# luo-yining/CFDBench

Hardware: NVIDIA H100
Metric: fno_rollout_steps_per_sec (higher is better)
Workload: dtype bf16

## Files before the change

cfdbench_b200/csrc/fno_block_fused.cu:

```cuda
#include "fno_common.cuh"
#include "tc_common.cuh"
#include "tc_tma.cuh"
#include <math.h>
#include <string.h>

namespace fno {

constexpr int kFzRows = 16;
constexpr int kFzChunks = kH / kFzRows;
constexpr int kFzWgRows = kFzRows / 2;
constexpr int kFzThreads = 9 * 32;
constexpr int kFzProdWarp = 8;
constexpr int kZK = 2 * kM2;
constexpr int kImgK = 2 * kKX;
constexpr size_t kYmImgBytes = 147456;
constexpr uint32_t kFzStage = 4 * 6144;
constexpr int kFzFFloats = 2 * (2 * kFzRows) * kImgK;
constexpr int kFzEFloats = 2 * kW * kZK;
constexpr uint32_t kFzZtFloats = kC * kZK;
constexpr uint32_t kLboF = (2 * kFzRows / 8) * 128;
constexpr uint32_t kLboE = (kW / 8) * 128;
constexpr uint32_t kLboO = (kC / 8) * 128;
constexpr uint32_t kFzBoxW = kW, kFzBoxH = 1, kFzBoxC = kC;
constexpr uint32_t kFzRowBytes = kFzBoxW * kFzBoxH * kFzBoxC * 2;
constexpr int kFzXSlots = 4;
constexpr uint32_t kFzW0Bytes = kC * kC * 2;

__host__ __device__ constexpr int fz_x_slot(int n) { return n % kFzXSlots; }
__host__ __device__ constexpr uint32_t fz_x_parity(int n) { return static_cast<uint32_t>(n / kFzXSlots) & 1u; }

struct FzSmem {
  alignas(1024) unsigned char x[2][kFzXSlots][kFzRowBytes];
  alignas(1024) unsigned char st[2][2][kFzRowBytes];
  alignas(128) unsigned char y[2][kFzStage];
  alignas(128) float zt[kFzRows][2][kFzZtFloats];
  alignas(128) float f_hi[kFzFFloats / 2];
  alignas(128) float f_lo[kFzFFloats / 2];
  alignas(128) float e_hi[kFzEFloats / 2];
  alignas(128) float e_lo[kFzEFloats / 2];
  alignas(128) unsigned char w0[3][kFzW0Bytes];
  alignas(16) float bias[kC];
  alignas(8) uint64_t y_full[2], y_free[2];
  alignas(8) uint64_t x_full[2][kFzXSlots];
};
static_assert(sizeof(FzSmem) <= 232448, "block_fused_kernel: shared memory over the per-block opt-in limit");

__device__ __forceinline__ uint32_t sw128_bf16_offset(int line, int e) {
  return static_cast<uint32_t>(line * 128 + ((((e >> 3) ^ line) & 7) << 4) + (e & 7) * 2);
}

__global__ void __launch_bounds__(kFzThreads, 1)
    block_fused_kernel(const __grid_constant__ CUtensorMap x_map, const __grid_constant__ CUtensorMap out_map,
                       const unsigned char* __restrict__ img, const float* __restrict__ w0t,
                       const float* __restrict__ bias, const float* __restrict__ etab, const float* __restrict__ ftab,
                       int batch) {
  extern __shared__ __align__(1024) unsigned char smem_raw[];
  FzSmem& sm = *reinterpret_cast<FzSmem*>(smem_raw);
  if ((smem_u32(smem_raw) & 1023u) != 0) __trap();
  const int tid = threadIdx.x, lane = tid & 31, warp = tc::warp_index_uniform();
  const int chunk = blockIdx.x % kFzChunks, b0 = blockIdx.x / kFzChunks, bstride = gridDim.x / kFzChunks;
  const int n_units = b0 < batch ? (batch - b0 + bstride - 1) / bstride : 0;

  if (tid == 0) {
    for (int i = 0; i < 2; ++i) {
      mbar_init(&sm.y_full[i], 1);
      mbar_init(&sm.y_free[i], 4);
      for (int s = 0; s < kFzXSlots; ++s) mbar_init(&sm.x_full[i][s], 1);
    }
    fence_mbar_init();
  }
  for (int e = tid; e < kFzFFloats / 2; e += kFzThreads) {
    sm.f_hi[e] = __ldg(ftab + chunk * kFzFFloats + e);
    sm.f_lo[e] = __ldg(ftab + chunk * kFzFFloats + kFzFFloats / 2 + e);
  }
  for (int e = tid; e < kFzEFloats / 2; e += kFzThreads) {
    sm.e_hi[e] = __ldg(etab + e);
    sm.e_lo[e] = __ldg(etab + kFzEFloats / 2 + e);
  }
  for (int e = tid; e < kC * kC; e += kFzThreads) {
    const int i = e / kC, o = e % kC;
    const float w = w0t[e];
    const __nv_bfloat16 t1 = __float2bfloat16_rn(w);
    const float r1 = w - __bfloat162float(t1);
    const __nv_bfloat16 t2 = __float2bfloat16_rn(r1);
    const __nv_bfloat16 t3 = __float2bfloat16_rn(r1 - __bfloat162float(t2));
    const uint32_t off = static_cast<uint32_t>(((i >> 3) * (kC / 8) + (o >> 3)) * 128 + (o & 7) * 16 + (i & 7) * 2);
    *reinterpret_cast<__nv_bfloat16*>(sm.w0[0] + off) = t1;
    *reinterpret_cast<__nv_bfloat16*>(sm.w0[1] + off) = t2;
    *reinterpret_cast<__nv_bfloat16*>(sm.w0[2] + off) = t3;
  }
  if (tid < kC) sm.bias[tid] = bias != nullptr ? bias[tid] : 0.f;
  tc::fence_proxy_async_smem();
  __syncthreads();
  pdl_wait();
  pdl_launch_dependents();

  if (warp == kFzProdWarp) {
    if (lane < 2) {
      const int s = lane;
      for (int u = 0; u < n_units; ++u) {
        const unsigned char* src = img + static_cast<size_t>(b0 + u * bstride) * kYmImgBytes;
        for (int pi = 0; pi < 3; ++pi) {
          const int p = s + 2 * pi, f = 3 * u + pi;
          if (f >= 1) mbar_wait(&sm.y_free[s], (f - 1) & 1);
          mbar_expect_tx(&sm.y_full[s], kFzStage);
          bulk_g2s(sm.y[s], src + p * (kFzStage / 2), kFzStage / 2, &sm.y_full[s]);
          bulk_g2s(sm.y[s] + kFzStage / 2, src + kYmImgBytes / 2 + p * (kFzStage / 2), kFzStage / 2, &sm.y_full[s]);
        }
      }
    }
    return;
  }

  const int g = warp >> 2, wq = warp & 3, q = lane & 3, t = tid & 127;
  const int m0 = 16 * wq + (lane >> 2);
  const int n_fills = kFzWgRows * n_units;
  auto x_fill = [&](int n) {
    const int u = n / kFzWgRows, r = n % kFzWgRows, s = fz_x_slot(n);
    mbar_expect_tx(&sm.x_full[g][s], kFzRowBytes);
    tma_load_3d(sm.x[g][s], &x_map, 0, kFzRows * chunk + g + 2 * r, (b0 + u * bstride) * kC, &sm.x_full[g][s]);
  };
  if (t == 0)
    for (int n = 0; n < kFzXSlots && n < n_fills; ++n) x_fill(n);
  const uint32_t w0_s = tc::smem_addr(sm.w0[0]);

  for (int u = 0; u < n_units; ++u) {
    const int b = b0 + u * bstride;
    for (int pi = 0; pi < 3; ++pi) {
      const int p = g + 2 * pi, f = 3 * u + pi;
      mbar_wait(&sm.y_full[g], f & 1);
      uint32_t a_hi[6][4], a_lo[6][4];
#pragma unroll
      for (int ks = 0; ks < kImgK / 8; ++ks)
#pragma unroll
        for (int r = 0; r < 4; ++r) {
          const int m = m0 + 8 * (r & 1), kk = 8 * ks + q + 4 * (r >> 1), o = m & 31;
          const uint32_t off = (m >> 5) * 6144 + kk * 128 + (((o >> 3) ^ (kk & 3)) << 5) + (o & 7) * 4;
          a_hi[ks][r] = *reinterpret_cast<const uint32_t*>(sm.y[g] + off);
          a_lo[ks][r] = *reinterpret_cast<const uint32_t*>(sm.y[g] + kFzStage / 2 + off);
        }
      float acc[16];
      tc::wg_fence();
#pragma unroll
      for (int pass = 0; pass < 3; ++pass) {
        const uint32_t fb = tc::smem_addr(pass == 2 ? sm.f_lo : sm.f_hi);
#pragma unroll
        for (int ks = 0; ks < kImgK / 8; ++ks)
          tc::wg_tf32_rs_n32(acc, pass == 1 ? a_lo[ks] : a_hi[ks], tc::make_smem_desc(fb + ks * 2 * kLboF, kLboF, 128),
                             (pass | ks) ? 1u : 0u);
      }
      tc::wg_commit();
      __syncwarp();
      if (lane == 0) mbar_arrive(&sm.y_free[g]);
      tc::wg_wait<0>();
      tc::wg_fence_acc(acc);
      if (pi == 0) tc::named_barrier(1, 256);
#pragma unroll
      for (int hh = 0; hh < 2; ++hh) {
        const int m = m0 + 8 * hh, ky = 2 * p + (m >> 5), o = m & 31;
#pragma unroll
        for (int i = 0; i < 4; ++i)
#pragma unroll
          for (int e = 0; e < 2; ++e) {
            float v = acc[4 * i + 2 * hh + e];
            if (ky == 0 && e == 1) v = sm.bias[o];
            float hi, lo;
            tc::split_tf32(v, hi, lo);
            const uint32_t off = tc::kmajor_offset(o, 2 * ky + e, kC) / 4;
            sm.zt[4 * i + q][0][off] = hi;
            sm.zt[4 * i + q][1][off] = lo;
          }
      }
    }
    tc::fence_proxy_async_smem();
    tc::named_barrier(1, 256);

    float acc[2][16];
#pragma unroll
    for (int r = 0; r <= kFzWgRows; ++r) {
      if (r < kFzWgRows) {
        const int n = kFzWgRows * u + r, hl = g + 2 * r;
        mbar_wait(&sm.x_full[g][fz_x_slot(n)], fz_x_parity(n));
        tc::wg_fence();
        const uint32_t a_e[3] = {tc::smem_addr(sm.e_hi), tc::smem_addr(sm.e_lo), tc::smem_addr(sm.e_hi)};
        const uint32_t b_z[3] = {tc::smem_addr(sm.zt[hl][0]), tc::smem_addr(sm.zt[hl][0]), tc::smem_addr(sm.zt[hl][1])};
#pragma unroll
        for (int pass = 0; pass < 3; ++pass)
#pragma unroll
          for (int ks = 0; ks < kZK / 8; ++ks)
            tc::wg_tf32_ss_n32(acc[r & 1], tc::make_smem_desc(a_e[pass] + ks * 2 * kLboE, kLboE, 128),
                               tc::make_smem_desc(b_z[pass] + ks * 2 * kLboO, kLboO, 128), (pass | ks) ? 1u : 0u);
        tc::wg_fence();
        const uint32_t a_x = tc::smem_addr(sm.x[g][fz_x_slot(n)]);
#pragma unroll
        for (int term = 0; term < 3; ++term)
#pragma unroll
          for (int ks = 0; ks < kC / 16; ++ks)
            tc::wg_bf16_ss_n32_mn_a(acc[r & 1], tc::make_smem_desc_sw128_mn(a_x + ks * 2048),
                                    tc::make_smem_desc(w0_s + term * kFzW0Bytes + ks * 2 * kLboO, kLboO, 128), 1u);
        tc::wg_commit();
      }
      if (r == 0) continue;
      const int rr = r - 1, h = kFzRows * chunk + g + 2 * rr;
      float* d = acc[rr & 1];
      if (r < kFzWgRows) {
        tc::wg_wait<1>();
      } else {
        tc::wg_wait<0>();
      }
      tc::wg_fence_acc(acc[rr & 1]);
      unsigned char* stile = sm.st[g][rr & 1];
#pragma unroll
      for (int i = 0; i < 4; ++i)
#pragma unroll
        for (int hh = 0; hh < 2; ++hh) {
          const float2 v = gelu_erf2(make_float2(d[4 * i + 2 * hh], d[4 * i + 2 * hh + 1]));
          const int w = m0 + 8 * hh, o = 8 * i + 2 * q;
          *reinterpret_cast<__nv_bfloat16*>(stile + sw128_bf16_offset(o, w)) = __float2bfloat16_rn(v.x);
          *reinterpret_cast<__nv_bfloat16*>(stile + sw128_bf16_offset(o + 1, w)) = __float2bfloat16_rn(v.y);
        }
      tc::fence_proxy_async_smem();
      if (t == 0) bulk_wait_group_read<0>();
      tc::named_barrier(2 + g, 128);
      if (t == 0) {
        tma_store_3d(&out_map, stile, 0, h, b * kC);
        bulk_commit_group();
        const int nf = kFzWgRows * u + rr + kFzXSlots;
        if (nf < n_fills) x_fill(nf);
      }
    }
  }
  if (t == 0) bulk_wait_group<0>();
}

void c2r_operand_table(float* host, double s0, double s1);

static float fz_round_tf32_host(double v) {
  float f = static_cast<float>(v);
  uint32_t u;
  memcpy(&u, &f, 4);
  u = (u + 0x1000u) & 0xffffe000u;
  memcpy(&f, &u, 4);
  return f;
}

struct FzTables {
  float* etab = nullptr;
  float* ftab = nullptr;
  int n_sm = 0;
  bool configured = false;
};
static FzTables g_fz[64];

static cudaError_t fz_ensure(int dev, cudaStream_t stream) {
  FzTables& t = g_fz[dev];
  if (t.configured) return cudaSuccess;
  const double two_pi = 6.283185307179586476925286766559;
  static float h_e[kFzEFloats];
  static float h_f[kFzChunks * kFzFFloats];
  c2r_operand_table(h_e, 1.0 / kHW, 2.0 / kHW);
  for (int c = 0; c < kFzChunks; ++c)
    for (int n = 0; n < 2 * kFzRows; ++n) {
      const int h = kFzRows * c + (n >> 1), ri = n & 1;
      for (int k = 0; k < kImgK; ++k) {
        const int rip = k & 1, kxi = 2 * ((k % 24) >> 1) + k / 24, kx = kxi < kM1 ? kxi : kxi + (kH - kKX);
        const double ang = two_pi * ((kx * h) % 64) / 64.0;
        const double val = (ri == rip) ? cos(ang) : (ri == 0 ? -sin(ang) : sin(ang));
        const float hi = fz_round_tf32_host(val);
        const uint32_t off = tc::kmajor_offset(n, k, 2 * kFzRows) / 4;
        h_f[c * kFzFFloats + off] = hi;
        h_f[c * kFzFFloats + kFzFFloats / 2 + off] = fz_round_tf32_host(val - static_cast<double>(hi));
      }
    }
  cudaError_t e = cudaMalloc(&t.etab, sizeof(h_e));
  if (e != cudaSuccess) return e;
  e = cudaMalloc(&t.ftab, sizeof(h_f));
  if (e != cudaSuccess) return e;
  e = cudaMemcpyAsync(t.etab, h_e, sizeof(h_e), cudaMemcpyHostToDevice, stream);
  if (e != cudaSuccess) return e;
  e = cudaMemcpyAsync(t.ftab, h_f, sizeof(h_f), cudaMemcpyHostToDevice, stream);
  if (e != cudaSuccess) return e;
  e = cudaStreamSynchronize(stream);
  if (e != cudaSuccess) return e;
  e = cudaFuncSetAttribute(block_fused_kernel, cudaFuncAttributeMaxDynamicSharedMemorySize, (int)sizeof(FzSmem));
  if (e != cudaSuccess) return e;
  e = cudaDeviceGetAttribute(&t.n_sm, cudaDevAttrMultiProcessorCount, dev);
  if (e != cudaSuccess) return e;
  t.configured = true;
  return cudaSuccess;
}

void block_fused_release(int dev) {
  if (dev < 0 || dev >= 64) return;
  FzTables& t = g_fz[dev];
  if (t.etab) cudaFree(t.etab);
  if (t.ftab) cudaFree(t.ftab);
  t = FzTables();
}

cudaError_t launch_block_fused(const void* ym_img, const void* x, const float* w0t, const float* bias, void* out, int batch,
                               cudaStream_t stream) {
  int dev = 0;
  cudaError_t e = cudaGetDevice(&dev);
  if (e != cudaSuccess) return e;
  if (dev < 0 || dev >= 64) return cudaErrorInvalidDevice;
  e = fz_ensure(dev, stream);
  if (e != cudaSuccess) return e;
  if ((reinterpret_cast<uintptr_t>(x) & 15) || (reinterpret_cast<uintptr_t>(ym_img) & 15) ||
      (reinterpret_cast<uintptr_t>(out) & 15))
    return cudaErrorMisalignedAddress;
  CUtensorMap x_map, out_map;
  const uint64_t planes = static_cast<uint64_t>(batch) * kC;
  e = make_tma_map_3d(&x_map, CU_TENSOR_MAP_DATA_TYPE_BFLOAT16, 2, x, kW, kH, planes, kFzBoxW, kFzBoxH, kFzBoxC);
  if (e != cudaSuccess) return e;
  e = make_tma_map_3d(&out_map, CU_TENSOR_MAP_DATA_TYPE_BFLOAT16, 2, out, kW, kH, planes, kFzBoxW, kFzBoxH, kFzBoxC);
  if (e != cudaSuccess) return e;
  const int slots_max = g_fz[dev].n_sm / kFzChunks;
  const int slots = batch < slots_max ? batch : slots_max;
  return launch_chained(block_fused_kernel, dim3(kFzChunks * slots), dim3(kFzThreads), sizeof(FzSmem), stream, x_map,
                        out_map, static_cast<const unsigned char*>(ym_img), w0t, bias,
                        static_cast<const float*>(g_fz[dev].etab), static_cast<const float*>(g_fz[dev].ftab), batch);
}

}
```

cfdbench_b200/csrc/tc_common.cuh:

```cuda
#pragma once
#include <cuda_runtime.h>
#include <stdint.h>

namespace fno {
namespace tc {

__device__ __forceinline__ uint32_t smem_addr(const void* p) {
  return static_cast<uint32_t>(__cvta_generic_to_shared(p));
}

__device__ __forceinline__ int warp_index_uniform() {
  return __shfl_sync(0xffffffffu, static_cast<int>(threadIdx.x >> 5), 0);
}

__device__ __forceinline__ void named_barrier(int id, int count) {
  asm volatile("bar.sync %0, %1;" ::"r"(id), "r"(count) : "memory");
}

__device__ __forceinline__ void fence_proxy_async_smem() {
  asm volatile("fence.proxy.async.shared::cta;" ::: "memory");
}

__device__ __forceinline__ uint64_t make_smem_desc(uint32_t saddr, uint32_t lbo_bytes, uint32_t sbo_bytes) {
  uint64_t d = 0;
  d |= static_cast<uint64_t>((saddr & 0x3FFFFu) >> 4);
  d |= static_cast<uint64_t>((lbo_bytes >> 4) & 0x3FFFu) << 16;
  d |= static_cast<uint64_t>((sbo_bytes >> 4) & 0x3FFFu) << 32;
  return d;
}
__device__ __forceinline__ uint64_t make_smem_desc_sw128(uint32_t saddr) {
  return make_smem_desc(saddr, 16, 1024) | (static_cast<uint64_t>(1) << 62);
}
__device__ __forceinline__ uint64_t make_smem_desc_sw128_mn(uint32_t saddr) {
  return make_smem_desc(saddr, 16, 1024) | (static_cast<uint64_t>(1) << 62);
}

__device__ __forceinline__ void wg_fence() { asm volatile("wgmma.fence.sync.aligned;" ::: "memory"); }
__device__ __forceinline__ void wg_commit() { asm volatile("wgmma.commit_group.sync.aligned;" ::: "memory"); }
template <int kPending>
__device__ __forceinline__ void wg_wait() { asm volatile("wgmma.wait_group.sync.aligned %0;" ::"n"(kPending) : "memory"); }
template <int N>
__device__ __forceinline__ void wg_fence_acc(float (&d)[N]) {
#pragma unroll
  for (int i = 0; i < N; ++i) asm volatile("" : "+f"(d[i])::"memory");
}

__device__ __forceinline__ void wg_tf32_ss_n32(float* d, uint64_t a, uint64_t b, uint32_t acc) {
  asm volatile(
      "{\n.reg .pred p;\nsetp.ne.b32 p, %18, 0;\n"
      "wgmma.mma_async.sync.aligned.m64n32k8.f32.tf32.tf32 {%0, %1, %2, %3, %4, %5, %6, %7, %8, %9, %10, %11, %12, %13, %14, %15}, %16, %17, p, 1, 1;\n}\n"
      : "+f"(d[0]), "+f"(d[1]), "+f"(d[2]), "+f"(d[3]), "+f"(d[4]), "+f"(d[5]), "+f"(d[6]), "+f"(d[7]), "+f"(d[8]), "+f"(d[9]), "+f"(d[10]), "+f"(d[11]), "+f"(d[12]), "+f"(d[13]), "+f"(d[14]), "+f"(d[15])
      : "l"(a), "l"(b), "r"(acc)
      : "memory");
}
__device__ __forceinline__ void wg_tf32_ss_n128(float* d, uint64_t a, uint64_t b, uint32_t acc) {
  asm volatile(
      "{\n.reg .pred p;\nsetp.ne.b32 p, %66, 0;\n"
      "wgmma.mma_async.sync.aligned.m64n128k8.f32.tf32.tf32 {%0, %1, %2, %3, %4, %5, %6, %7, %8, %9, %10, %11, %12, %13, %14, %15, %16, %17, %18, %19, %20, %21, %22, %23, %24, %25, %26, %27, %28, %29, %30, %31, %32, %33, %34, %35, %36, %37, %38, %39, %40, %41, %42, %43, %44, %45, %46, %47, %48, %49, %50, %51, %52, %53, %54, %55, %56, %57, %58, %59, %60, %61, %62, %63}, %64, %65, p, 1, 1;\n}\n"
      : "+f"(d[0]), "+f"(d[1]), "+f"(d[2]), "+f"(d[3]), "+f"(d[4]), "+f"(d[5]), "+f"(d[6]), "+f"(d[7]), "+f"(d[8]), "+f"(d[9]), "+f"(d[10]), "+f"(d[11]), "+f"(d[12]), "+f"(d[13]), "+f"(d[14]), "+f"(d[15]), "+f"(d[16]), "+f"(d[17]), "+f"(d[18]), "+f"(d[19]), "+f"(d[20]), "+f"(d[21]), "+f"(d[22]), "+f"(d[23]), "+f"(d[24]), "+f"(d[25]), "+f"(d[26]), "+f"(d[27]), "+f"(d[28]), "+f"(d[29]), "+f"(d[30]), "+f"(d[31]), "+f"(d[32]), "+f"(d[33]), "+f"(d[34]), "+f"(d[35]), "+f"(d[36]), "+f"(d[37]), "+f"(d[38]), "+f"(d[39]), "+f"(d[40]), "+f"(d[41]), "+f"(d[42]), "+f"(d[43]), "+f"(d[44]), "+f"(d[45]), "+f"(d[46]), "+f"(d[47]), "+f"(d[48]), "+f"(d[49]), "+f"(d[50]), "+f"(d[51]), "+f"(d[52]), "+f"(d[53]), "+f"(d[54]), "+f"(d[55]), "+f"(d[56]), "+f"(d[57]), "+f"(d[58]), "+f"(d[59]), "+f"(d[60]), "+f"(d[61]), "+f"(d[62]), "+f"(d[63])
      : "l"(a), "l"(b), "r"(acc)
      : "memory");
}
__device__ __forceinline__ void wg_bf16_ss_n72(float* d, uint64_t a, uint64_t b, uint32_t acc) {
  asm volatile(
      "{\n.reg .pred p;\nsetp.ne.b32 p, %38, 0;\n"
      "wgmma.mma_async.sync.aligned.m64n72k16.f32.bf16.bf16 {%0, %1, %2, %3, %4, %5, %6, %7, %8, %9, %10, %11, %12, %13, %14, %15, %16, %17, %18, %19, %20, %21, %22, %23, %24, %25, %26, %27, %28, %29, %30, %31, %32, %33, %34, %35}, %36, %37, p, 1, 1, 0, 0;\n}\n"
      : "+f"(d[0]), "+f"(d[1]), "+f"(d[2]), "+f"(d[3]), "+f"(d[4]), "+f"(d[5]), "+f"(d[6]), "+f"(d[7]), "+f"(d[8]), "+f"(d[9]), "+f"(d[10]), "+f"(d[11]), "+f"(d[12]), "+f"(d[13]), "+f"(d[14]), "+f"(d[15]), "+f"(d[16]), "+f"(d[17]), "+f"(d[18]), "+f"(d[19]), "+f"(d[20]), "+f"(d[21]), "+f"(d[22]), "+f"(d[23]), "+f"(d[24]), "+f"(d[25]), "+f"(d[26]), "+f"(d[27]), "+f"(d[28]), "+f"(d[29]), "+f"(d[30]), "+f"(d[31]), "+f"(d[32]), "+f"(d[33]), "+f"(d[34]), "+f"(d[35])
      : "l"(a), "l"(b), "r"(acc)
      : "memory");
}
__device__ __forceinline__ void wg_bf16_ss_n32_mn_a(float* d, uint64_t a, uint64_t b, uint32_t acc) {
  asm volatile(
      "{\n.reg .pred p;\nsetp.ne.b32 p, %18, 0;\n"
      "wgmma.mma_async.sync.aligned.m64n32k16.f32.bf16.bf16 {%0, %1, %2, %3, %4, %5, %6, %7, %8, %9, %10, %11, %12, %13, %14, %15}, %16, %17, p, 1, 1, 1, 0;\n}\n"
      : "+f"(d[0]), "+f"(d[1]), "+f"(d[2]), "+f"(d[3]), "+f"(d[4]), "+f"(d[5]), "+f"(d[6]), "+f"(d[7]), "+f"(d[8]), "+f"(d[9]), "+f"(d[10]), "+f"(d[11]), "+f"(d[12]), "+f"(d[13]), "+f"(d[14]), "+f"(d[15])
      : "l"(a), "l"(b), "r"(acc)
      : "memory");
}
__device__ __forceinline__ void wg_tf32_rs_n32(float* d, const uint32_t* a, uint64_t b, uint32_t acc) {
  asm volatile(
      "{\n.reg .pred p;\nsetp.ne.b32 p, %21, 0;\n"
      "wgmma.mma_async.sync.aligned.m64n32k8.f32.tf32.tf32 {%0, %1, %2, %3, %4, %5, %6, %7, %8, %9, %10, %11, %12, %13, %14, %15}, {%16, %17, %18, %19}, %20, p, 1, 1;\n}\n"
      : "+f"(d[0]), "+f"(d[1]), "+f"(d[2]), "+f"(d[3]), "+f"(d[4]), "+f"(d[5]), "+f"(d[6]), "+f"(d[7]), "+f"(d[8]), "+f"(d[9]), "+f"(d[10]), "+f"(d[11]), "+f"(d[12]), "+f"(d[13]), "+f"(d[14]), "+f"(d[15])
      : "r"(a[0]), "r"(a[1]), "r"(a[2]), "r"(a[3]), "l"(b), "r"(acc)
      : "memory");
}
__device__ __forceinline__ void wg_tf32_rs_n48(float* d, const uint32_t* a, uint64_t b, uint32_t acc) {
  asm volatile(
      "{\n.reg .pred p;\nsetp.ne.b32 p, %29, 0;\n"
      "wgmma.mma_async.sync.aligned.m64n48k8.f32.tf32.tf32 {%0, %1, %2, %3, %4, %5, %6, %7, %8, %9, %10, %11, %12, %13, %14, %15, %16, %17, %18, %19, %20, %21, %22, %23}, {%24, %25, %26, %27}, %28, p, 1, 1;\n}\n"
      : "+f"(d[0]), "+f"(d[1]), "+f"(d[2]), "+f"(d[3]), "+f"(d[4]), "+f"(d[5]), "+f"(d[6]), "+f"(d[7]), "+f"(d[8]), "+f"(d[9]), "+f"(d[10]), "+f"(d[11]), "+f"(d[12]), "+f"(d[13]), "+f"(d[14]), "+f"(d[15]), "+f"(d[16]), "+f"(d[17]), "+f"(d[18]), "+f"(d[19]), "+f"(d[20]), "+f"(d[21]), "+f"(d[22]), "+f"(d[23])
      : "r"(a[0]), "r"(a[1]), "r"(a[2]), "r"(a[3]), "l"(b), "r"(acc)
      : "memory");
}
__device__ __forceinline__ void wg_tf32_rs_n64(float* d, const uint32_t* a, uint64_t b, uint32_t acc) {
  asm volatile(
      "{\n.reg .pred p;\nsetp.ne.b32 p, %37, 0;\n"
      "wgmma.mma_async.sync.aligned.m64n64k8.f32.tf32.tf32 {%0, %1, %2, %3, %4, %5, %6, %7, %8, %9, %10, %11, %12, %13, %14, %15, %16, %17, %18, %19, %20, %21, %22, %23, %24, %25, %26, %27, %28, %29, %30, %31}, {%32, %33, %34, %35}, %36, p, 1, 1;\n}\n"
      : "+f"(d[0]), "+f"(d[1]), "+f"(d[2]), "+f"(d[3]), "+f"(d[4]), "+f"(d[5]), "+f"(d[6]), "+f"(d[7]), "+f"(d[8]), "+f"(d[9]), "+f"(d[10]), "+f"(d[11]), "+f"(d[12]), "+f"(d[13]), "+f"(d[14]), "+f"(d[15]), "+f"(d[16]), "+f"(d[17]), "+f"(d[18]), "+f"(d[19]), "+f"(d[20]), "+f"(d[21]), "+f"(d[22]), "+f"(d[23]), "+f"(d[24]), "+f"(d[25]), "+f"(d[26]), "+f"(d[27]), "+f"(d[28]), "+f"(d[29]), "+f"(d[30]), "+f"(d[31])
      : "r"(a[0]), "r"(a[1]), "r"(a[2]), "r"(a[3]), "l"(b), "r"(acc)
      : "memory");
}

__host__ __device__ constexpr uint32_t kmajor_offset(int row, int k, int rows) {
  return static_cast<uint32_t>(((k >> 2) * (rows >> 3) + (row >> 3)) * 128 + (row & 7) * 16 + (k & 3) * 4);
}
__device__ __forceinline__ float round_tf32(float x) {
  return __uint_as_float((__float_as_uint(x) + 0x1000u) & 0xffffe000u);
}
__device__ __forceinline__ void split_tf32(float x, float& hi, float& lo) {
  hi = round_tf32(x);
  lo = round_tf32(x - hi);
}

}
}
```

Before: 1256.

## Feed wgmma A operands from registers and store GELU output with stmatrix

The constant E table is loaded once into per-thread register fragments, and the bf16 x tile is read with ldmatrix.trans each row, so both the tf32 and the bf16 wgmma run in register-sourced (RS) form instead of reading A from shared-memory descriptors. The shared E arrays are removed, which frees shared memory. The GELU epilogue now packs bf16x2 pairs and writes them with stmatrix.trans instead of scalar swizzled stores. This raises register pressure (E fragments plus a double-buffered x fragment) and adds an ldmatrix step ahead of the MMAs.

```diff
diff --git a/cfdbench_b200/csrc/fno_block_fused.cu b/cfdbench_b200/csrc/fno_block_fused.cu
--- a/cfdbench_b200/csrc/fno_block_fused.cu
+++ b/cfdbench_b200/csrc/fno_block_fused.cu
@@ -19,7 +19,6 @@
 constexpr int kFzEFloats = 2 * kW * kZK;
 constexpr uint32_t kFzZtFloats = kC * kZK;
 constexpr uint32_t kLboF = (2 * kFzRows / 8) * 128;
-constexpr uint32_t kLboE = (kW / 8) * 128;
 constexpr uint32_t kLboO = (kC / 8) * 128;
 constexpr uint32_t kFzBoxW = kW, kFzBoxH = 1, kFzBoxC = kC;
 constexpr uint32_t kFzRowBytes = kFzBoxW * kFzBoxH * kFzBoxC * 2;
@@ -36,8 +35,6 @@
   alignas(128) float zt[kFzRows][2][kFzZtFloats];
   alignas(128) float f_hi[kFzFFloats / 2];
   alignas(128) float f_lo[kFzFFloats / 2];
-  alignas(128) float e_hi[kFzEFloats / 2];
-  alignas(128) float e_lo[kFzEFloats / 2];
   alignas(128) unsigned char w0[3][kFzW0Bytes];
   alignas(16) float bias[kC];
   alignas(8) uint64_t y_full[2], y_free[2];
@@ -72,10 +69,6 @@
   for (int e = tid; e < kFzFFloats / 2; e += kFzThreads) {
     sm.f_hi[e] = __ldg(ftab + chunk * kFzFFloats + e);
     sm.f_lo[e] = __ldg(ftab + chunk * kFzFFloats + kFzFFloats / 2 + e);
-  }
-  for (int e = tid; e < kFzEFloats / 2; e += kFzThreads) {
-    sm.e_hi[e] = __ldg(etab + e);
-    sm.e_lo[e] = __ldg(etab + kFzEFloats / 2 + e);
   }
   for (int e = tid; e < kC * kC; e += kFzThreads) {
     const int i = e / kC, o = e % kC;
@@ -123,6 +116,16 @@
   if (t == 0)
     for (int n = 0; n < kFzXSlots && n < n_fills; ++n) x_fill(n);
   const uint32_t w0_s = tc::smem_addr(sm.w0[0]);
+  uint32_t e_frag[2][kZK / 8][4];
+#pragma unroll
+  for (int hl = 0; hl < 2; ++hl)
+#pragma unroll
+    for (int ks = 0; ks < kZK / 8; ++ks)
+#pragma unroll
+      for (int j = 0; j < 4; ++j) {
+        const uint32_t off = tc::kmajor_offset(m0 + 8 * (j & 1), 8 * ks + q + 4 * (j >> 1), kW) / 4;
+        e_frag[hl][ks][j] = __float_as_uint(__ldg(etab + hl * (kFzEFloats / 2) + off));
+      }
 
   for (int u = 0; u < n_units; ++u) {
     const int b = b0 + u * bstride;
@@ -176,28 +179,32 @@
     tc::named_barrier(1, 256);
 
     float acc[2][16];
+    uint32_t x_frag[2][kC / 16][4];
 #pragma unroll
     for (int r = 0; r <= kFzWgRows; ++r) {
       if (r < kFzWgRows) {
         const int n = kFzWgRows * u + r, hl = g + 2 * r;
         mbar_wait(&sm.x_full[g][fz_x_slot(n)], fz_x_parity(n));
+        const uint32_t a_x = tc::smem_addr(sm.x[g][fz_x_slot(n)]);
+#pragma unroll
+        for (int ks = 0; ks < kC / 16; ++ks)
+          tc::ldmatrix_x4_trans(x_frag[r & 1][ks], a_x + sw128_bf16_offset(16 * ks + 8 * (lane >> 4) + (lane & 7),
+                                                                             16 * wq + 8 * ((lane >> 3) & 1)));
         tc::wg_fence();
-        const uint32_t a_e[3] = {tc::smem_addr(sm.e_hi), tc::smem_addr(sm.e_lo), tc::smem_addr(sm.e_hi)};
         const uint32_t b_z[3] = {tc::smem_addr(sm.zt[hl][0]), tc::smem_addr(sm.zt[hl][0]), tc::smem_addr(sm.zt[hl][1])};
 #pragma unroll
         for (int pass = 0; pass < 3; ++pass)
 #pragma unroll
           for (int ks = 0; ks < kZK / 8; ++ks)
-            tc::wg_tf32_ss_n32(acc[r & 1], tc::make_smem_desc(a_e[pass] + ks * 2 * kLboE, kLboE, 128),
+            tc::wg_tf32_rs_n32(acc[r & 1], e_frag[pass == 1][ks],
                                tc::make_smem_desc(b_z[pass] + ks * 2 * kLboO, kLboO, 128), (pass | ks) ? 1u : 0u);
         tc::wg_fence();
-        const uint32_t a_x = tc::smem_addr(sm.x[g][fz_x_slot(n)]);
 #pragma unroll
         for (int term = 0; term < 3; ++term)
 #pragma unroll
           for (int ks = 0; ks < kC / 16; ++ks)
-            tc::wg_bf16_ss_n32_mn_a(acc[r & 1], tc::make_smem_desc_sw128_mn(a_x + ks * 2048),
-                                    tc::make_smem_desc(w0_s + term * kFzW0Bytes + ks * 2 * kLboO, kLboO, 128), 1u);
+            tc::wg_bf16_rs_n32(acc[r & 1], x_frag[r & 1][ks],
+                               tc::make_smem_desc(w0_s + term * kFzW0Bytes + ks * 2 * kLboO, kLboO, 128), 1u);
         tc::wg_commit();
       }
       if (r == 0) continue;
@@ -211,14 +218,19 @@
       tc::wg_fence_acc(acc[rr & 1]);
       unsigned char* stile = sm.st[g][rr & 1];
 #pragma unroll
-      for (int i = 0; i < 4; ++i)
-#pragma unroll
-        for (int hh = 0; hh < 2; ++hh) {
-          const float2 v = gelu_erf2(make_float2(d[4 * i + 2 * hh], d[4 * i + 2 * hh + 1]));
-          const int w = m0 + 8 * hh, o = 8 * i + 2 * q;
-          *reinterpret_cast<__nv_bfloat16*>(stile + sw128_bf16_offset(o, w)) = __float2bfloat16_rn(v.x);
-          *reinterpret_cast<__nv_bfloat16*>(stile + sw128_bf16_offset(o + 1, w)) = __float2bfloat16_rn(v.y);
+      for (int i2 = 0; i2 < 2; ++i2) {
+        uint32_t v[4];
+#pragma unroll
+        for (int j = 0; j < 4; ++j) {
+          const int i = 2 * i2 + (j >> 1), hh = j & 1;
+          const float2 y = gelu_erf2(make_float2(d[4 * i + 2 * hh], d[4 * i + 2 * hh + 1]));
+          const __nv_bfloat162 p = __floats2bfloat162_rn(y.x, y.y);
+          v[j] = *reinterpret_cast<const uint32_t*>(&p);
         }
+        tc::stmatrix_x4_trans(tc::smem_addr(stile) + sw128_bf16_offset(16 * i2 + 8 * (lane >> 4) + (lane & 7),
+                                                                       16 * wq + 8 * ((lane >> 3) & 1)),
+                              v);
+      }
       tc::fence_proxy_async_smem();
       if (t == 0) bulk_wait_group_read<0>();
       tc::named_barrier(2 + g, 128);
diff --git a/cfdbench_b200/csrc/tc_common.cuh b/cfdbench_b200/csrc/tc_common.cuh
--- a/cfdbench_b200/csrc/tc_common.cuh
+++ b/cfdbench_b200/csrc/tc_common.cuh
@@ -29,9 +29,6 @@
   return d;
 }
 __device__ __forceinline__ uint64_t make_smem_desc_sw128(uint32_t saddr) {
-  return make_smem_desc(saddr, 16, 1024) | (static_cast<uint64_t>(1) << 62);
-}
-__device__ __forceinline__ uint64_t make_smem_desc_sw128_mn(uint32_t saddr) {
   return make_smem_desc(saddr, 16, 1024) | (static_cast<uint64_t>(1) << 62);
 }
 
@@ -69,18 +66,18 @@
       : "l"(a), "l"(b), "r"(acc)
       : "memory");
 }
-__device__ __forceinline__ void wg_bf16_ss_n32_mn_a(float* d, uint64_t a, uint64_t b, uint32_t acc) {
-  asm volatile(
-      "{\n.reg .pred p;\nsetp.ne.b32 p, %18, 0;\n"
-      "wgmma.mma_async.sync.aligned.m64n32k16.f32.bf16.bf16 {%0, %1, %2, %3, %4, %5, %6, %7, %8, %9, %10, %11, %12, %13, %14, %15}, %16, %17, p, 1, 1, 1, 0;\n}\n"
-      : "+f"(d[0]), "+f"(d[1]), "+f"(d[2]), "+f"(d[3]), "+f"(d[4]), "+f"(d[5]), "+f"(d[6]), "+f"(d[7]), "+f"(d[8]), "+f"(d[9]), "+f"(d[10]), "+f"(d[11]), "+f"(d[12]), "+f"(d[13]), "+f"(d[14]), "+f"(d[15])
-      : "l"(a), "l"(b), "r"(acc)
-      : "memory");
-}
 __device__ __forceinline__ void wg_tf32_rs_n32(float* d, const uint32_t* a, uint64_t b, uint32_t acc) {
   asm volatile(
       "{\n.reg .pred p;\nsetp.ne.b32 p, %21, 0;\n"
       "wgmma.mma_async.sync.aligned.m64n32k8.f32.tf32.tf32 {%0, %1, %2, %3, %4, %5, %6, %7, %8, %9, %10, %11, %12, %13, %14, %15}, {%16, %17, %18, %19}, %20, p, 1, 1;\n}\n"
+      : "+f"(d[0]), "+f"(d[1]), "+f"(d[2]), "+f"(d[3]), "+f"(d[4]), "+f"(d[5]), "+f"(d[6]), "+f"(d[7]), "+f"(d[8]), "+f"(d[9]), "+f"(d[10]), "+f"(d[11]), "+f"(d[12]), "+f"(d[13]), "+f"(d[14]), "+f"(d[15])
+      : "r"(a[0]), "r"(a[1]), "r"(a[2]), "r"(a[3]), "l"(b), "r"(acc)
+      : "memory");
+}
+__device__ __forceinline__ void wg_bf16_rs_n32(float* d, const uint32_t* a, uint64_t b, uint32_t acc) {
+  asm volatile(
+      "{\n.reg .pred p;\nsetp.ne.b32 p, %21, 0;\n"
+      "wgmma.mma_async.sync.aligned.m64n32k16.f32.bf16.bf16 {%0, %1, %2, %3, %4, %5, %6, %7, %8, %9, %10, %11, %12, %13, %14, %15}, {%16, %17, %18, %19}, %20, p, 1, 1, 0;\n}\n"
       : "+f"(d[0]), "+f"(d[1]), "+f"(d[2]), "+f"(d[3]), "+f"(d[4]), "+f"(d[5]), "+f"(d[6]), "+f"(d[7]), "+f"(d[8]), "+f"(d[9]), "+f"(d[10]), "+f"(d[11]), "+f"(d[12]), "+f"(d[13]), "+f"(d[14]), "+f"(d[15])
       : "r"(a[0]), "r"(a[1]), "r"(a[2]), "r"(a[3]), "l"(b), "r"(acc)
       : "memory");
@@ -102,6 +99,18 @@
       : "memory");
 }
 
+__device__ __forceinline__ void ldmatrix_x4_trans(uint32_t (&r)[4], uint32_t saddr) {
+  asm volatile("ldmatrix.sync.aligned.m8n8.x4.trans.shared.b16 {%0, %1, %2, %3}, [%4];"
+               : "=r"(r[0]), "=r"(r[1]), "=r"(r[2]), "=r"(r[3])
+               : "r"(saddr)
+               : "memory");
+}
+__device__ __forceinline__ void stmatrix_x4_trans(uint32_t saddr, const uint32_t (&r)[4]) {
+  asm volatile("stmatrix.sync.aligned.m8n8.x4.trans.shared.b16 [%0], {%1, %2, %3, %4};" ::"r"(saddr), "r"(r[0]),
+               "r"(r[1]), "r"(r[2]), "r"(r[3])
+               : "memory");
+}
+
 __host__ __device__ constexpr uint32_t kmajor_offset(int row, int k, int rows) {
   return static_cast<uint32_t>(((k >> 2) * (rows >> 3) + (row >> 3)) * 128 + (row & 7) * 16 + (k & 3) * 4);
 }
```

After: 1296, median of 6. 1.03x the previous value.
